# MPEGGroup/mpeg-pcc-tmc2

Measured on AMD Instinct MI355X. Metric: encoder patch+image-gen frames/sec, longdress_vox10 32-frame GOF, higher is better.
Workload: dtype int32/f64

## Files before the change

### mpeg-pcc-tmc2_amd/csrc/patches.hip

```cpp
#include <algorithm>
#include <cmath>

#include "internal.h"
#include "union_find.h"

namespace tmc2 {
namespace {

using Uf = UnionFind<false>;

constexpr uint32_t kNoLabel = 0xFFFFFFFFu;
constexpr uint32_t kFar     = 0xFFFFFFFFu;

struct PatchDev {
  int32_t u1, v1, d1;
  int32_t sizeU, sizeV, sizeU0, sizeV0;
  int32_t axN, axT, axB, mode;
  int32_t blockBase;
  int64_t depthOff;
  int64_t occOff;
};

__device__ __forceinline__ int coordOf( const Pt p, int axis ) { return axis == 0 ? p.x : ( axis == 1 ? p.y : p.z ); }

// ... 35 lines not shown
  for ( int j = 0; j < K; ++j ) {
    const uint32_t v = nb[j];
    if ( v == u ) continue;
    const uint4* rv  = reinterpret_cast<const uint4*>( knn + size_t( v ) * K );
    bool         hit = false;
#pragma unroll
    for ( int t = 0; t < K / 4; ++t ) {
      const uint4 r = rv[t];
      hit |= ( r.x == u ) | ( r.y == u ) | ( r.z == u ) | ( r.w == u );
    }
    m |= hit ? ( 1u << j ) : 0u;
  }
  mutual[u] = uint16_t( m );
}

template <int K>
__global__ __launch_bounds__( 256 ) void ccInitKernel( const uint32_t* __restrict__ knn, const uint16_t* __restrict__ mutual,
                                                        const uint8_t* __restrict__ partition, const uint8_t* __restrict__ raw,
                                                        const uint32_t* __restrict__ perm, bool chunked, uint32_t n,
                                                        uint32_t* __restrict__ parent, uint32_t* __restrict__ lab,
                                                        uint32_t* __restrict__ ccCount ) {
  const uint32_t i = pointOfLane( perm, chunked, n );
  if ( i >= n ) return;
  lab[i]        = kNoLabel;
  ccCount[i]    = 0;
  uint32_t best = i;
  if ( raw[i] ) {
    uint32_t      bestPrio = ufPriority( i ), m = mutual[i];
    const uint8_t pi       = partition[i];
    while ( m ) {
      const int j = __ffs( int( m ) ) - 1;
      m &= m - 1;
      const uint32_t v = knn[size_t( i ) * K + j];
      if ( ufPriority( v ) < bestPrio && raw[v] && partition[v] == pi ) {
        best     = v;
        bestPrio = ufPriority( v );
      }
    }
  }
  parent[i] = best;
}

template <int K>
__global__ __launch_bounds__( 256 ) void ccUnionKernel( const uint32_t* __restrict__ knn, const uint16_t* __restrict__ mutual,
                                                         const uint8_t* __restrict__ partition,
                                                         const uint8_t* __restrict__ raw, const uint32_t* __restrict__ perm,
                                                         bool chunked, uint32_t n, uint32_t* __restrict__ parent, int precheck,
                                                         bool agent ) {
  const uint32_t u = pointOfLane( perm, chunked, n );
  if ( u >= n || !raw[u] ) return;
  uint32_t m = mutual[u];
  if ( !m ) return;
  const uint8_t   pu  = partition[u];
  const uint32_t* row = knn + size_t( u ) * K;
  while ( m ) {
    const int j = __ffs( int( m ) ) - 1;
    m &= m - 1;
    const uint32_t v = row[j];
    if ( v > u || !raw[v] || partition[v] != pu ) continue;
    if ( precheck && Uf::sameSetStale( parent, u, v, agent ) ) continue;
    Uf::unite( parent, u, v, 0u, agent );
  }
}

template <int K>
__global__ __launch_bounds__( 256 ) void ccCheckKernel( const uint32_t* __restrict__ knn, const uint16_t* __restrict__ mutual,
                                                         const uint8_t* __restrict__ partition, const uint8_t* __restrict__ raw,
                                                         uint32_t n, uint32_t* parent, uint32_t* __restrict__ bad ) {
  const uint32_t u = blockIdx.x * blockDim.x + threadIdx.x;
  if ( u >= n || !raw[u] ) return;
  const uint32_t p = __hip_atomic_load( &parent[u], __ATOMIC_RELAXED, __HIP_MEMORY_SCOPE_AGENT );
  if ( p != u && ( p >= n || !raw[p] || partition[p] != partition[u] || ufPriority( p ) >= ufPriority( u ) ) ) atomicAdd( &bad[0], 1u );
  const uint32_t ru = Uf::rootCoherent( parent, u, n );
  if ( ru == kUfBroken ) {
    atomicAdd( &bad[0], 1u );
    return;
  }
  uint32_t m = mutual[u];
  while ( m ) {
    const int j = __ffs( int( m ) ) - 1;
    m &= m - 1;
    const uint32_t v = knn[size_t( u ) * K + j];
    if ( v > u || !raw[v] || partition[v] != partition[u] ) continue;
    if ( Uf::rootCoherent( parent, v, n ) != ru ) atomicAdd( &bad[1], 1u );
  }
}

__global__ __launch_bounds__( 256 ) void ccFlattenSeedKernel( const uint8_t* __restrict__ raw, const uint32_t* __restrict__ dist,
                                                               uint32_t thrDetection, uint32_t n,
                                                               uint32_t* __restrict__ parent, uint32_t* __restrict__ root,
                                                               uint32_t* __restrict__ lab, bool agent ) {
  const uint32_t u    = chunkedIndex();
  const int      lane = threadIdx.x & 63;
  uint32_t       r    = kNoLabel;
  bool           seed = false;
  if ( u < n && raw[u] ) {
    r       = Uf::find( parent, u, agent ).root;
    root[u] = r;
    seed    = dist[u] > thrDetection;
  }
  unsigned long long todo = __ballot( seed );
  while ( todo ) {
    const int                leader = __ffsll( (long long)todo ) - 1;
    const uint32_t           key    = __shfl( r, leader, 64 );
    const unsigned long long same   = __ballot( seed && r == key );
    if ( lane == leader && loadStaleOk( &lab[key], agent ) > u )
      atomicMin( &lab[key], u );
    todo &= ~same;
  }
}

template <int K>
__global__ __launch_bounds__( 256 ) void ccRelaxKernel( const uint32_t* __restrict__ knn, const uint16_t* __restrict__ mutual,
                                                         const uint8_t* __restrict__ partition,
                                                         const uint8_t* __restrict__ raw, const uint32_t* __restrict__ parent,
                                                         const uint32_t* __restrict__ perm, bool chunked, uint32_t n,
                                                         uint32_t* __restrict__ lab, uint32_t* __restrict__ changed, uint32_t token,
                                                         bool agent ) {
  const uint32_t u = pointOfLane( perm, chunked, n );
  if ( u >= n || !raw[u] ) return;
  uint32_t m = ~uint32_t( mutual[u] ) & ( ( 1u << K ) - 1u );
  if ( !m ) return;
  const uint32_t ru = parent[u];
  const uint32_t lu = loadStaleOk( &lab[ru], agent );
  if ( lu == kNoLabel ) return;
  const uint8_t   pu  = partition[u];
  const uint32_t* row = knn + size_t( u ) * K;
  bool            any = false;
  while ( m ) {
    const int j = __ffs( int( m ) ) - 1;
    m &= m - 1;
    const uint32_t v = row[j];
    if ( v == u || !raw[v] || partition[v] != pu ) continue;
    const uint32_t rv = parent[v];
    if ( rv != ru && loadStaleOk( &lab[rv], agent ) > lu &&
         atomicMin( &lab[rv], lu ) > lu )
      any = true;
  }
  if ( any ) *changed = token;
}

constexpr uint32_t kRawCounters = 16;
__global__ __launch_bounds__( 256 ) void patchBoundsInitKernel( uint32_t P, int32_t* __restrict__ bbox, int32_t* __restrict__ minUv,
                                                                 int32_t* __restrict__ patchStat, uint32_t* __restrict__ rawCount ) {
  const uint32_t p = blockIdx.x * blockDim.x + threadIdx.x;
  if ( p < kRawCounters ) rawCount[p * 32] = 0;
  if ( p >= P ) return;
#pragma unroll
  for ( int d = 0; d < 3; ++d ) {
    bbox[6 * p + d]     = 0x7FFFFFFF;
    bbox[6 * p + 3 + d] = 0;
  }
  minUv[2 * p] = minUv[2 * p + 1] = 0x7F7F7F7F;
  patchStat[2 * p] = patchStat[2 * p + 1] = 0;
}

__global__ __launch_bounds__( 256 ) void ccLabelCountKernel( const uint8_t* __restrict__ raw, const uint32_t* __restrict__ parent,
                                                              const uint32_t* __restrict__ lab, uint32_t n, uint32_t minCount,
                                                              uint32_t* __restrict__ label, uint32_t* __restrict__ ccCount ) {
  const uint32_t i    = chunkedIndex();
  const int      lane = threadIdx.x & 63;
  const uint32_t l    = ( i < n && raw[i] ) ? lab[parent[i]] : kNoLabel;
  if ( i < n ) label[i] = l;
  unsigned long long todo = __ballot( l != kNoLabel );
  while ( todo ) {
    const int                leader = __ffsll( (long long)todo ) - 1;
    const uint32_t           key    = __shfl( l, leader, 64 );
    const unsigned long long same   = __ballot( l == key );
    if ( lane == leader && loadStaleOk( &ccCount[key] ) < minCount ) atomicAdd( &ccCount[key], uint32_t( __popcll( same ) ) );
    todo &= ~same;
  }
}

__global__ __launch_bounds__( 256 ) void ccSeedFlagKernel( const uint32_t* __restrict__ label,
                                                            const uint32_t* __restrict__ ccCount, uint32_t minCount,
                                                            uint32_t n, uint32_t* __restrict__ flag ) {
  const uint32_t i = chunkedIndex();
  if ( i < n ) flag[i] = ( label[i] == i && ccCount[i] >= minCount ) ? 1u : 0u;
}

__global__ __launch_bounds__( 256 ) void ccAssignKernel( const uint32_t* __restrict__ label,
                                                          const uint32_t* __restrict__ ccCount,
                                                          const uint32_t* __restrict__ rank,
                                                          const uint8_t* __restrict__ partition, uint32_t minCount,
                                                          uint32_t n, int32_t* __restrict__ pointPatch,
                                                          int32_t* __restrict__ patchView ) {
  const uint32_t i = chunkedIndex();
  if ( i >= n ) return;
  const uint32_t l = label[i];
  int32_t        p = -1;
  if ( l != kNoLabel && ccCount[l] >= minCount ) {
    p = int32_t( rank[l] );
    if ( l == i ) patchView[p] = partition[i];
  }
  pointPatch[i] = p;
}

constexpr int kAggSlots = 128;
template <int FIELDS>
struct PatchAgg {
  int32_t key[kAggSlots];
  int32_t val[kAggSlots][FIELDS];
};
template <int FIELDS, int MINS>
__device__ __forceinline__ void aggInit( PatchAgg<FIELDS>& t ) {
  for ( int i = threadIdx.x; i < kAggSlots; i += blockDim.x ) {
    t.key[i] = -1;
// ... 28 lines not shown
}
template <int FIELDS, int MINS>
__device__ __forceinline__ void aggFlush( PatchAgg<FIELDS>& t, int32_t* __restrict__ out ) {
  __syncthreads();
  for ( int i = threadIdx.x; i < kAggSlots * FIELDS; i += blockDim.x ) {
    const int     slot = i / FIELDS, f = i % FIELDS;
    const int32_t k    = t.key[slot];
    if ( k < 0 ) continue;
    if ( f < MINS )
      lazyAtomicMin( &out[FIELDS * k + f], t.val[slot][f] );
    else
      lazyAtomicMax( &out[FIELDS * k + f], t.val[slot][f] );
  }
}

__global__ __launch_bounds__( 256 ) void patchMinUvKernel( const Pt* __restrict__ pts, const int32_t* __restrict__ pointPatch,
                                                            const int32_t* __restrict__ patchView, uint32_t n,
                                                            int32_t* __restrict__ minUv ) {
  __shared__ PatchAgg<2> agg;
  aggInit<2, 2>( agg );
  const uint32_t i = chunkedIndex();
  const int32_t  p = i < n ? pointPatch[i] : -1;
  if ( p >= 0 ) {
    const int view = patchView[p] % 3;
    const int axT = view == 0 ? 2 : ( view == 1 ? 2 : 0 ), axB = view == 0 ? 1 : ( view == 1 ? 0 : 1 );
    const Pt  q    = pts[i];
    const int uv[2] = {coordOf( q, axT ), coordOf( q, axB )};
    aggAdd<2, 2>( agg, p, uv, minUv );
  }
  aggFlush<2, 2>( agg, minUv );
}

__global__ __launch_bounds__( 256 ) void patchTrimBboxKernel( const Pt* __restrict__ pts, const int32_t* __restrict__ patchView,
                                                               const int32_t* __restrict__ minUv, int splitting,
                                                               int maxPatchSize, uint32_t n,
                                                               int32_t* __restrict__ pointPatch, int32_t* __restrict__ bbox ) {
  __shared__ PatchAgg<6> agg;
  aggInit<6, 3>( agg );
  const uint32_t i = chunkedIndex();
  int32_t        p = i < n ? pointPatch[i] : -1;
  if ( p >= 0 ) {
    const Pt q = pts[i];
    if ( splitting ) {
      const int view = patchView[p] % 3;
      const int axT = view == 0 ? 2 : ( view == 1 ? 2 : 0 ), axB = view == 0 ? 1 : ( view == 1 ? 0 : 1 );
      if ( !( coordOf( q, axT ) - minUv[2 * p] < maxPatchSize && coordOf( q, axB ) - minUv[2 * p + 1] < maxPatchSize ) ) {
        pointPatch[i] = -1;
        p             = -1;
      }
    }
    if ( p >= 0 ) {
      const int box[6] = {q.x, q.y, q.z, q.x, q.y, q.z};
      aggAdd<6, 3>( agg, p, box, bbox );
    }
  }
  aggFlush<6, 3>( agg, bbox );
}

__global__ __launch_bounds__( 256 ) void patchDepth0Kernel( const Pt* __restrict__ pts, const int32_t* __restrict__ pointPatch,
                                                             const PatchDev* __restrict__ patches, uint32_t n,
                                                             int64_t roundDepthBase,
                                                             unsigned long long* __restrict__ map64 ) {
  const uint32_t i = chunkedIndex();
  if ( i >= n ) return;
  const int32_t p = pointPatch[i];
  if ( p < 0 ) return;
  const PatchDev pd = patches[p];
  const Pt       q  = pts[i];
  const int      d = coordOf( q, pd.axN ), u = coordOf( q, pd.axT ) - pd.u1, v = coordOf( q, pd.axB ) - pd.v1;
  const size_t   px  = size_t( pd.depthOff - roundDepthBase ) + size_t( v ) * pd.sizeU + u;
  const unsigned long long val = ( (unsigned long long)uint32_t( d + 1 ) << 32 ) | i;
  if ( pd.mode == 0 )
    atomicMin( &map64[px], val );
  else
    atomicMax( &map64[px], val );
}

__global__ __launch_bounds__( 256 ) void patchInitTileKernel( const PatchDev* __restrict__ patches,
// ... 50 lines not shown
  if ( depth != INF ) {
    const int     dir = 1 - 2 * pd.mode;
    const int16_t a   = int16_t( abs( depth - pk ) );
    const int16_t b   = int16_t( int16_t( surfaceThickness ) + dir * depth );
    const int16_t c   = int16_t( dir * pd.d1 + int16_t( maxAllowedDepth ) );
    if ( a > 32 || b > c ) {
      depth = INF;
      src   = 0xFFFFFFFFu;
    }
  }
  d0tmp[px] = depth;
  d1tmp[px] = depth;
  d0src[px] = src;
}

__global__ __launch_bounds__( 256 ) void patchDepth1Kernel( const Pt* __restrict__ pts, const uint8_t* __restrict__ rgb4,
                                                             const int32_t* __restrict__ pointPatch,
                                                             const PatchDev* __restrict__ patches, uint32_t n,
                                                             int64_t roundDepthBase, int surfaceThickness,
                                                             const int32_t* __restrict__ d0tmp,
                                                             const uint32_t* __restrict__ d0src, int32_t* __restrict__ d1tmp ) {
  const uint32_t i = chunkedIndex();
  if ( i >= n ) return;
  const int32_t p = pointPatch[i];
  if ( p < 0 ) return;
  const PatchDev pd = patches[p];
  const Pt       q  = pts[i];
  const int      d = coordOf( q, pd.axN ), u = coordOf( q, pd.axT ) - pd.u1, v = coordOf( q, pd.axB ) - pd.v1;
  const size_t   px = size_t( pd.depthOff - roundDepthBase ) + size_t( v ) * pd.sizeU + u;
  const int      z0 = d0tmp[px];
  if ( !( z0 < 32767 ) ) return;
  const int     dir   = 1 - 2 * pd.mode;
  const int16_t delta = int16_t( dir * ( d - z0 ) );
  if ( !( delta <= int16_t( surfaceThickness ) && delta >= 0 ) ) return;
  const uchar4 ci = reinterpret_cast<const uchar4*>( rgb4 )[i];
  const uchar4 c0 = reinterpret_cast<const uchar4*>( rgb4 )[d0src[px]];
  if ( !( abs( int( c0.x ) - int( ci.x ) ) < 128 && abs( int( c0.y ) - int( ci.y ) ) < 128 &&
// ... 58 lines not shown
    anyValid[threadIdx.x >> 6] = __popcll( m );
    tileMax[threadIdx.x >> 6]  = mx;
  }
  __syncthreads();
  if ( threadIdx.x == 0 ) {
    const int count = anyValid[0] + anyValid[1] + anyValid[2] + anyValid[3];
    occupancy[size_t( pd.occOff ) + size_t( bv ) * pd.sizeU0 + bu] = count ? 1 : 0;
    if ( count ) {
      const int tmx = max( max( tileMax[0], tileMax[1] ), max( tileMax[2], tileMax[3] ) );
      if ( tmx > loadStaleOk( &patchStat[2 * p] ) ) atomicMax( &patchStat[2 * p], tmx );
      atomicAdd( &patchStat[2 * p + 1], count );
    }
  }
}

__global__ __launch_bounds__( 256 ) void rawDistanceKernel( const Pt* __restrict__ pts, uint32_t n,
                                                             const uint32_t* __restrict__ bitmap, int bitmapBits,
                                                             const int* __restrict__ offsets, int nOffsets,
                                                             uint32_t thrSelection, uint32_t* __restrict__ dist,
                                                             uint8_t* __restrict__ raw, uint32_t* __restrict__ rawCount ) {
  const uint32_t i = chunkedIndex();
  bool           isRaw = false;
  if ( i < n ) {
    const Pt  q    = pts[i];
    const int size = 1 << bitmapBits;
    uint32_t  best = kFar;
    for ( int o = 0; o < nOffsets; ++o ) {
      const int packed = offsets[o];
      const int dx = ( packed & 0xFF ) - 128, dy = ( ( packed >> 8 ) & 0xFF ) - 128, dz = ( ( packed >> 16 ) & 0xFF ) - 128;
      const int x = q.x + dx, y = q.y + dy, z = q.z + dz;
      if ( x < 0 || y < 0 || z < 0 || x >= size || y >= size || z >= size ) continue;
      const size_t bit = size_t( x ) + ( size_t( y ) << bitmapBits ) + ( size_t( z ) << ( 2 * bitmapBits ) );
      if ( bitmap[bit >> 5] & ( 1u << ( bit & 31 ) ) ) {
        best = uint32_t( packed >> 24 );
        break;
      }
    }
    dist[i] = best;
    isRaw   = best > thrSelection;
    raw[i]  = isRaw ? 1 : 0;
  }
  __shared__ uint32_t wgRaw;
  if ( threadIdx.x == 0 ) wgRaw = 0;
  __syncthreads();
  const unsigned long long m = __ballot( isRaw );
  if ( ( threadIdx.x & 63 ) == 0 && m ) atomicAdd( &wgRaw, uint32_t( __popcll( m ) ) );
  __syncthreads();
  if ( threadIdx.x == 0 && wgRaw ) atomicAdd( &rawCount[( blockIdx.x % kRawCounters ) * 32], wgRaw );
}

}

int ensureMutualMask( tmc2_frame* f ) {
  if ( f->haveMutual ) return TMC2_OK;
  const uint32_t n = uint32_t( f->n );
  TMC2_TRY( f->d_mutual.alloc( n ) );
  StageScope stage( f->ctx, "k:ccMutualMask" );
  const PassOrder order  = passOrder( f, "MUTUAL_ORDER" );
  const uint32_t  blocks = ( n + 255 ) / 256;
  hipLaunchKernelGGL( ccMutualMaskKernel<16>, dim3( order.chunked ? chunkedGrid( blocks ) : blocks ), dim3( 256 ), 0, f->ctx->stream, f->d_knn.p,
                      order.perm, order.chunked, n, f->d_mutual.p );
  TMC2_HIP( hipGetLastError() );
  f->haveMutual = true;
// ... 36 lines not shown
    std::vector<std::pair<int, int>> tmp;
    for ( int dz = -R; dz <= R; ++dz )
      for ( int dy = -R; dy <= R; ++dy )
        for ( int dx = -R; dx <= R; ++dx ) {
          const int d2 = dx * dx + dy * dy + dz * dz;
          if ( d2 <= probeR2 ) tmp.emplace_back( d2, ( dx + 128 ) | ( ( dy + 128 ) << 8 ) | ( ( dz + 128 ) << 16 ) );
        }
    std::sort( tmp.begin(), tmp.end() );
    for ( auto& t : tmp ) offsets.push_back( t.second | ( t.first << 24 ) );
  }
  int bitmapBits = 1;
  while ( ( 1 << bitmapBits ) <= int( f->geoMax ) ) ++bitmapBits;
  const size_t bitmapWords = ( size_t( 1 ) << ( 3 * bitmapBits ) ) >> 5;
  TMC2_TRY( ctx->voxelBitmap.alloc( bitmapWords ) );

  DevBuf<uint32_t> d_label, d_ccCount, d_flag, d_rank, d_dist, d_small, d_tilePatch, d_d0src, d_parent, d_root, d_lab;
  DevBuf<uint8_t>  d_raw;
  DevBuf<int32_t>  d_pointPatch, d_minUv, d_bbox, d_patchStat, d_d0tmp, d_d1tmp;
  DevBuf<PatchDev> d_patches;
  DevBuf<unsigned long long> d_map64;
  TMC2_TRY( d_label.alloc( n ) );
  TMC2_TRY( d_parent.alloc( n ) );
  TMC2_TRY( d_root.alloc( n ) );
  TMC2_TRY( d_lab.alloc( n ) );
  TMC2_TRY( d_ccCount.alloc( n ) );
  TMC2_TRY( d_flag.alloc( n ) );
  TMC2_TRY( d_rank.alloc( n ) );
  TMC2_TRY( d_dist.alloc( n ) );
  TMC2_TRY( d_raw.alloc( n ) );
  TMC2_TRY( d_pointPatch.alloc( n ) );
  TMC2_TRY( d_small.alloc( 16 ) );
  const int* d_offsets = ctx->constTable( ( uint64_t( 0x5339 ) << 32 ) | uint64_t( probeR2 ), offsets );
  if ( !d_offsets ) return TMC2_E_HIP;
  TMC2_TRY( fillRegions( ctx, {{ctx->voxelBitmap.p, bitmapWords * 4, 0},
                               {d_raw.p, n, 1},
                               {d_dist.p, size_t( n ) * 4, 0xFF},
                               {d_small.p, 64, 0}} ) );

  f->patches.clear();
  f->patchesChanged();
  f->depthCount = 0;
  f->occCount   = 0;
  const dim3  blk( 256 ), grdN( chunkedGrid( ( n + 255 ) / 256 ) );
  uint32_t    rawCount = n, relaxToken = 0;
  int        rounds   = 0;
  TMC2_TRY( ensureMutualMask( f ) );
  DevBuf<uint16_t>& d_mutual   = f->d_mutual;
  const bool        agentScope = unionAgentScope( f->ctx );
  const PassOrder order   = passOrder( f, "MUTUAL_ORDER" );
  const bool      chunked = order.chunked;
  const uint32_t* perm    = order.perm;
  while ( rawCount > 0 ) {
    StageScope cc( ctx, "patches_cc" );
    hipLaunchKernelGGL( ccInitKernel<16>, grdN, blk, 0, s, f->d_knn.p, d_mutual.p, f->d_partition.p, d_raw.p, perm, chunked, n, d_parent.p,
                        d_lab.p, d_ccCount.p );
    {
      StageScope kt( ctx, "k:ccUnion" );
      hipLaunchKernelGGL( ccUnionKernel<16>, grdN, blk, 0, s, f->d_knn.p, d_mutual.p, f->d_partition.p, d_raw.p, perm, chunked, n,
                          d_parent.p, unionPrecheck( f->ctx ), agentScope );
      kt.end();
      if ( unionCheck( f->ctx ) ) {
        TMC2_HIP( hipMemsetAsync( d_small.p + 8, 0, 8, s ) );
        hipLaunchKernelGGL( ccCheckKernel<16>, grdN, blk, 0, s, f->d_knn.p, d_mutual.p, f->d_partition.p, d_raw.p, n,
                            d_parent.p, d_small.p + 8 );
        TMC2_TRY( unionCheckResult( s, d_small.p + 8, "segmentPatches: union-find invariant broken in round " + std::to_string( rounds ) ) );
      }
      hipLaunchKernelGGL( ccFlattenSeedKernel, grdN, blk, 0, s, d_raw.p, d_dist.p, thrDet, n, d_parent.p, d_root.p, d_lab.p,
                          agentScope );
    }
    uint32_t P = 0;
    for ( int guard = 0; guard < 1 << 20; ++guard ) {
      StageScope kt( ctx, "k:ccRelax" );
      for ( int b = 0; b < 3; ++b )
        hipLaunchKernelGGL( ccRelaxKernel<16>, grdN, blk, 0, s, f->d_knn.p, d_mutual.p, f->d_partition.p, d_raw.p,
                            d_root.p, perm, chunked, n, d_lab.p, d_small.p, ++relaxToken, agentScope );
      kt.end();
      hipLaunchKernelGGL( ccLabelCountKernel, grdN, blk, 0, s, d_raw.p, d_root.p, d_lab.p, n,
                          uint32_t( sp->minPointCountPerCCPatchSegmentation ), d_label.p, d_ccCount.p );
      hipLaunchKernelGGL( ccSeedFlagKernel, grdN, blk, 0, s, d_label.p, d_ccCount.p,
                          uint32_t( sp->minPointCountPerCCPatchSegmentation ), n, d_flag.p );
      volatile uint32_t* answer = ctx->answerLine( tmc2_ctx::kAnswerPatchRound );
      TMC2_TRY( exclusiveScanU32( ctx, d_flag.p, d_rank.p, n, d_small.p + 1, ScanAnswer{answer, d_small.p, 1} ) );
      TMC2_HIP( hipStreamSynchronize( s ) );
      P = answer[0];
      if ( answer[1] != relaxToken ) break;
      TMC2_HIP( hipMemsetAsync( d_ccCount.p, 0, size_t( n ) * 4, s ) );
    }
    cc.end();
    if ( P == 0 ) break;
    StageScope build( ctx, "patches_build" );
    TMC2_TRY( d_minUv.alloc( 2 * size_t( P ) ) );
    TMC2_TRY( d_bbox.alloc( 7 * size_t( P ) ) );
    const size_t statWords = 2 * size_t( P ) + size_t( kRawCounters ) * 32;
    TMC2_TRY( d_patchStat.alloc( statWords ) );
    int32_t*  d_view     = d_bbox.p + 6 * size_t( P );
    uint32_t* d_rawCount = reinterpret_cast<uint32_t*>( d_patchStat.p + 2 * size_t( P ) );
    TMC2_TRY( d_patches.alloc( P ) );
    hipLaunchKernelGGL( ccAssignKernel, grdN, blk, 0, s, d_label.p, d_ccCount.p, d_rank.p, f->d_partition.p,
                        uint32_t( sp->minPointCountPerCCPatchSegmentation ), n, d_pointPatch.p, d_view );
    hipLaunchKernelGGL( patchBoundsInitKernel, dim3( ( P + 255 ) / 256 ), blk, 0, s, P, d_bbox.p, d_minUv.p, d_patchStat.p,
                        d_rawCount );
    if ( sp->enablePatchSplitting )
      hipLaunchKernelGGL( patchMinUvKernel, grdN, blk, 0, s, f->d_pts.p, d_pointPatch.p, d_view, n, d_minUv.p );
    hipLaunchKernelGGL( patchTrimBboxKernel, grdN, blk, 0, s, f->d_pts.p, d_view, d_minUv.p,
                        sp->enablePatchSplitting, sp->maxPatchSize, n, d_pointPatch.p, d_bbox.p );
    int32_t* h_records = ctx->hostRecords.get<int32_t>( std::max<size_t>( 7 * size_t( P ) + statWords, size_t( 1 ) << 16 ) );
    if ( !h_records ) {
      setError( "segmentPatches: hipHostMalloc failed" );
      return TMC2_E_HIP;
    }
    const int32_t* h_bbox = h_records;
    TMC2_HIP( hipMemcpyAsync( h_records, d_bbox.p, 7 * size_t( P ) * 4, hipMemcpyDeviceToHost, s ) );
    const int32_t* h_view = h_bbox + 6 * size_t( P );
    TMC2_HIP( hipStreamSynchronize( s ) );
    for ( uint32_t p = 0; p < P; ++p )
      if ( h_bbox[6 * p] > h_bbox[6 * p + 3] ) {
        f->patches.clear();
        f->depthCount = f->occCount = 0;
        f->havePatches              = false;
        setError( "segmentPatches: patch splitting with maxPatchSize=%d keeps no point of a connected component (round %d); "
// ... 51 lines not shown
    const size_t pdBytes = ( size_t( P ) * sizeof( PatchDev ) + 15 ) & ~size_t( 15 );
    uint8_t*     h_tables = ctx->hostTables.get<uint8_t>( std::max<size_t>( pdBytes + size_t( tiles ) * 4, size_t( 1 ) << 20 ) );
    if ( !h_tables ) {
      setError( "segmentPatches: hipHostMalloc failed" );
      return TMC2_E_HIP;
    }
    memcpy( h_tables, h_pd, size_t( P ) * sizeof( PatchDev ) );
    uint32_t* h_tilePatch = reinterpret_cast<uint32_t*>( h_tables + pdBytes );
    for ( uint32_t p = 0, at = 0; p < P; ++p )
      for ( uint32_t b = uint32_t( h_pd[p].sizeU0 ) * uint32_t( h_pd[p].sizeV0 ); b > 0; --b ) h_tilePatch[at++] = p;
    TMC2_TRY( f->growPools() );
    TMC2_TRY( d_map64.alloc( roundArea ) );
    TMC2_TRY( d_d0tmp.alloc( roundArea ) );
    TMC2_TRY( d_d1tmp.alloc( roundArea ) );
    TMC2_TRY( d_d0src.alloc( roundArea ) );
    TMC2_TRY( d_tilePatch.alloc( tiles ) );
    TMC2_HIP( hipMemcpyAsync( d_patches.p, h_tables, size_t( P ) * sizeof( PatchDev ), hipMemcpyHostToDevice, s ) );
    TMC2_HIP( hipMemcpyAsync( d_tilePatch.p, h_tilePatch, size_t( tiles ) * 4, hipMemcpyHostToDevice, s ) );
    hipLaunchKernelGGL( patchInitTileKernel, dim3( tiles ), blk, 0, s, d_patches.p, d_tilePatch.p, roundDepthBase, occRes,
                        d_map64.p );
    hipLaunchKernelGGL( patchDepth0Kernel, grdN, blk, 0, s, f->d_pts.p, d_pointPatch.p, d_patches.p, n, roundDepthBase,
                        d_map64.p );
    hipLaunchKernelGGL( patchFilterTileKernel, dim3( tiles ), blk, 0, s, d_patches.p, d_tilePatch.p, d_map64.p,
                        roundDepthBase, occRes, sp->surfaceThickness, sp->maxAllowedDepth, d_d0tmp.p, d_d1tmp.p,
                        d_d0src.p );
    if ( sp->surfaceThickness > 0 )
      hipLaunchKernelGGL( patchDepth1Kernel, grdN, blk, 0, s, f->d_pts.p, f->d_rgb.p, d_pointPatch.p, d_patches.p, n,
                          roundDepthBase, sp->surfaceThickness, d_d0tmp.p, d_d0src.p, d_d1tmp.p );
    hipLaunchKernelGGL( patchResampleTileKernel, dim3( tiles ), blk, 0, s, d_patches.p, d_tilePatch.p, roundDepthBase,
                        occRes, d_d0tmp.p, d_d1tmp.p, bitmapBits, ctx->voxelBitmap.p, f->d_depth0.p, f->d_depth1.p,
                        f->d_occupancy.p, d_patchStat.p );
    int32_t* h_stat = h_records + 7 * size_t( P );
    hipLaunchKernelGGL( rawDistanceKernel, grdN, blk, 0, s, f->d_pts.p, n, ctx->voxelBitmap.p, bitmapBits, d_offsets,
                        int( offsets.size() ), thrSel, d_dist.p, d_raw.p, d_rawCount );
    TMC2_HIP( hipMemcpyAsync( h_stat, d_patchStat.p, statWords * 4, hipMemcpyDeviceToHost, s ) );
    TMC2_HIP( hipStreamSynchronize( s ) );
    const uint32_t rawBefore = rawCount;
    rawCount = 0;
    for ( uint32_t c = 0; c < kRawCounters; ++c ) rawCount += uint32_t( h_stat[2 * size_t( P ) + size_t( c ) * 32] );
    build.end();
    if ( rawCount >= rawBefore ) {
      f->patches.clear();
      f->depthCount = f->occCount = 0;
      f->havePatches              = false;
      setError( "segmentPatches: round %d took no point off the raw list (%u left); the reference does not terminate on this input",
                rounds, rawCount );
      return TMC2_E_UNSUPPORTED;
    }
    for ( uint32_t p = 0; p < P; ++p ) {
      tmc2_patch& T = f->patches[patchBase + p];
      const int   sizeD = h_stat[2 * p];
      T.sizeDPixel      = sizeD;
      const int bits    = std::min( sp->geometryBitDepth3D, sp->geometryBitDepth2D );
      const int L       = sp->minLevel;
      const int sd      = std::min( ( 1 << bits ) - 1, sizeD );
      const int bitsD   = bits - int( std::log2( L ) );
      int       q       = sd == 0 ? 0 : ( ( sd - 1 ) / L + 1 );
      q                 = std::min( q, ( 1 << bitsD ) - 1 );
      T.sizeD           = q == 0 ? 0 : ( q * L - 1 );
      T.d0Count         = h_stat[2 * p + 1];
      T.eomAndD1Count   = 0;
    }
    ++rounds;
  }
  TMC2_HIP( hipGetLastError() );
  f->rounds      = rounds;
  f->havePatches = true;
  f->geometryBitDepth3D = sp->geometryBitDepth3D;
  return TMC2_OK;
}

}

extern "C" int tmc2_selftest_components( tmc2_ctx* ctx, const uint32_t* d_knn, const uint8_t* d_partition, const uint8_t* d_raw,
                                         const uint32_t* d_perm, uint64_t n64, uint32_t* d_root, uint32_t* d_bad ) {
  using namespace tmc2;
  if ( !ctx || !d_knn || !d_partition || !d_raw || !d_root || !d_bad || n64 == 0 || n64 > 0x0FFFFFFFull ) {
    setError( "selftest_components: invalid argument (null pointer, no point, or more than 2^28 - 1 points)" );
    return TMC2_E_INVALID;
// ... 6 lines not shown
  TMC2_TRY( d_mutual.alloc( n ) );
  TMC2_TRY( d_parent.alloc( n ) );
  TMC2_TRY( d_lab.alloc( n ) );
  TMC2_TRY( d_ccCount.alloc( n ) );
  TMC2_TRY( d_dist.alloc( n ) );
  TMC2_TRY( fillRegions( ctx, {{d_parent.p, size_t( n ) * 4, 0}, {d_mutual.p, size_t( n ) * 2, 0}, {d_dist.p, size_t( n ) * 4, 0}} ) );
  const auto      option  = ctxOption( ctx, "MUTUAL_ORDER" );
  const char      o       = option ? ( *option )[0] : 'c';
  const bool      chunked = o != 'i';
  const uint32_t* perm    = o == 't' ? d_perm : nullptr;
  const uint32_t  blocks  = ( n + 255 ) / 256;
  const dim3      blk( 256 ), grdN( chunkedGrid( blocks ) );
  const bool      agentScope = unionAgentScope( ctx );
  hipLaunchKernelGGL( ccMutualMaskKernel<16>, dim3( chunked ? chunkedGrid( blocks ) : blocks ), dim3( 256 ), 0, s, d_knn, perm, chunked, n,
                      d_mutual.p );
  hipLaunchKernelGGL( ccInitKernel<16>, grdN, blk, 0, s, d_knn, d_mutual.p, d_partition, d_raw, perm, chunked, n, d_parent.p, d_lab.p,
                      d_ccCount.p );
  hipLaunchKernelGGL( ccUnionKernel<16>, grdN, blk, 0, s, d_knn, d_mutual.p, d_partition, d_raw, perm, chunked, n, d_parent.p,
                      unionPrecheck( ctx ), agentScope );
  if ( unionCheck( ctx ) )
    hipLaunchKernelGGL( ccCheckKernel<16>, grdN, blk, 0, s, d_knn, d_mutual.p, d_partition, d_raw, n, d_parent.p, d_bad );
  hipLaunchKernelGGL( ccFlattenSeedKernel, grdN, blk, 0, s, d_raw, d_dist.p, 0xFFFFFFFFu, n, d_parent.p, d_root, d_lab.p, agentScope );
  TMC2_HIP( hipGetLastError() );
  return TMC2_OK;
}
```

Before: 194.8.

## Compact raw points into a list so later segmentation rounds process only them

After each patch round, raw points are compacted through a flag scan and scatter into a ping-pong list with a position map. Later rounds launch the CC, assignment, bbox, depth and raw-distance kernels over that list only, not all n points. The per-block raw counters are replaced by a scan total read from a host-visible answer line, and the patch and tile tables are merged into one upload. This cuts work in rounds after the first, at the cost of an extra scan and scatter per round, indirect indexing, and added bookkeeping complexity.

```diff
diff --git a/mpeg-pcc-tmc2_amd/csrc/patches.hip b/mpeg-pcc-tmc2_amd/csrc/patches.hip
--- a/mpeg-pcc-tmc2_amd/csrc/patches.hip
+++ b/mpeg-pcc-tmc2_amd/csrc/patches.hip
@@ -73,13 +73,26 @@
   mutual[u] = uint16_t( m );
 }
 
-template <int K>
+template <bool LIST>
+__device__ __forceinline__ uint32_t roundPoint( const uint32_t* __restrict__ list, uint32_t count, uint32_t n ) {
+  const uint32_t j = chunkedIndex();
+  if ( LIST ) return j < count ? list[j] : n;
+  return j < n ? j : n;
+}
+template <bool LIST>
+__device__ __forceinline__ uint32_t roundPoint( const uint32_t* __restrict__ list, uint32_t count, const uint32_t* __restrict__ perm,
+                                                bool chunked, uint32_t n ) {
+  return LIST ? roundPoint<true>( list, count, n ) : pointOfLane( perm, chunked, n );
+}
+
+template <bool LIST, int K>
 __global__ __launch_bounds__( 256 ) void ccInitKernel( const uint32_t* __restrict__ knn, const uint16_t* __restrict__ mutual,
                                                         const uint8_t* __restrict__ partition, const uint8_t* __restrict__ raw,
-                                                        const uint32_t* __restrict__ perm, bool chunked, uint32_t n,
+                                                        const uint32_t* __restrict__ perm, bool chunked,
+                                                        const uint32_t* __restrict__ list, uint32_t count, uint32_t n,
                                                         uint32_t* __restrict__ parent, uint32_t* __restrict__ lab,
                                                         uint32_t* __restrict__ ccCount ) {
-  const uint32_t i = pointOfLane( perm, chunked, n );
+  const uint32_t i = roundPoint<LIST>( list, count, perm, chunked, n );
   if ( i >= n ) return;
   lab[i]        = kNoLabel;
   ccCount[i]    = 0;
@@ -100,13 +113,13 @@
   parent[i] = best;
 }
 
-template <int K>
+template <bool LIST, int K>
 __global__ __launch_bounds__( 256 ) void ccUnionKernel( const uint32_t* __restrict__ knn, const uint16_t* __restrict__ mutual,
                                                          const uint8_t* __restrict__ partition,
                                                          const uint8_t* __restrict__ raw, const uint32_t* __restrict__ perm,
-                                                         bool chunked, uint32_t n, uint32_t* __restrict__ parent, int precheck,
-                                                         bool agent ) {
-  const uint32_t u = pointOfLane( perm, chunked, n );
+                                                         bool chunked, const uint32_t* __restrict__ list, uint32_t count, uint32_t n,
+                                                         uint32_t* __restrict__ parent, int precheck, bool agent ) {
+  const uint32_t u = roundPoint<LIST>( list, count, perm, chunked, n );
   if ( u >= n || !raw[u] ) return;
   uint32_t m = mutual[u];
   if ( !m ) return;
@@ -122,11 +135,14 @@
   }
 }
 
-template <int K>
+template <bool LIST, int K>
 __global__ __launch_bounds__( 256 ) void ccCheckKernel( const uint32_t* __restrict__ knn, const uint16_t* __restrict__ mutual,
                                                          const uint8_t* __restrict__ partition, const uint8_t* __restrict__ raw,
-                                                         uint32_t n, uint32_t* parent, uint32_t* __restrict__ bad ) {
-  const uint32_t u = blockIdx.x * blockDim.x + threadIdx.x;
+                                                         const uint32_t* __restrict__ list, uint32_t count, uint32_t n, uint32_t* parent,
+                                                         uint32_t* __restrict__ bad ) {
+  const uint32_t at = blockIdx.x * blockDim.x + threadIdx.x;
+  if ( at >= count ) return;
+  const uint32_t u = LIST ? list[at] : at;
   if ( u >= n || !raw[u] ) return;
   const uint32_t p = __hip_atomic_load( &parent[u], __ATOMIC_RELAXED, __HIP_MEMORY_SCOPE_AGENT );
   if ( p != u && ( p >= n || !raw[p] || partition[p] != partition[u] || ufPriority( p ) >= ufPriority( u ) ) ) atomicAdd( &bad[0], 1u );
@@ -145,11 +161,12 @@
   }
 }
 
+template <bool LIST>
 __global__ __launch_bounds__( 256 ) void ccFlattenSeedKernel( const uint8_t* __restrict__ raw, const uint32_t* __restrict__ dist,
-                                                               uint32_t thrDetection, uint32_t n,
-                                                               uint32_t* __restrict__ parent, uint32_t* __restrict__ root,
-                                                               uint32_t* __restrict__ lab, bool agent ) {
-  const uint32_t u    = chunkedIndex();
+                                                               uint32_t thrDetection, const uint32_t* __restrict__ list,
+                                                               uint32_t count, uint32_t n, uint32_t* __restrict__ parent,
+                                                               uint32_t* __restrict__ root, uint32_t* __restrict__ lab, bool agent ) {
+  const uint32_t u    = roundPoint<LIST>( list, count, n );
   const int      lane = threadIdx.x & 63;
   uint32_t       r    = kNoLabel;
   bool           seed = false;
@@ -169,14 +186,15 @@
   }
 }
 
-template <int K>
+template <bool LIST, int K>
 __global__ __launch_bounds__( 256 ) void ccRelaxKernel( const uint32_t* __restrict__ knn, const uint16_t* __restrict__ mutual,
                                                          const uint8_t* __restrict__ partition,
                                                          const uint8_t* __restrict__ raw, const uint32_t* __restrict__ parent,
-                                                         const uint32_t* __restrict__ perm, bool chunked, uint32_t n,
+                                                         const uint32_t* __restrict__ perm, bool chunked,
+                                                         const uint32_t* __restrict__ list, uint32_t count, uint32_t n,
                                                          uint32_t* __restrict__ lab, uint32_t* __restrict__ changed, uint32_t token,
                                                          bool agent ) {
-  const uint32_t u = pointOfLane( perm, chunked, n );
+  const uint32_t u = roundPoint<LIST>( list, count, perm, chunked, n );
   if ( u >= n || !raw[u] ) return;
   uint32_t m = ~uint32_t( mutual[u] ) & ( ( 1u << K ) - 1u );
   if ( !m ) return;
@@ -199,11 +217,9 @@
   if ( any ) *changed = token;
 }
 
-constexpr uint32_t kRawCounters = 16;
 __global__ __launch_bounds__( 256 ) void patchBoundsInitKernel( uint32_t P, int32_t* __restrict__ bbox, int32_t* __restrict__ minUv,
-                                                                 int32_t* __restrict__ patchStat, uint32_t* __restrict__ rawCount ) {
+                                                                 int32_t* __restrict__ patchStat ) {
   const uint32_t p = blockIdx.x * blockDim.x + threadIdx.x;
-  if ( p < kRawCounters ) rawCount[p * 32] = 0;
   if ( p >= P ) return;
 #pragma unroll
   for ( int d = 0; d < 3; ++d ) {
@@ -214,10 +230,12 @@
   patchStat[2 * p] = patchStat[2 * p + 1] = 0;
 }
 
+template <bool LIST>
 __global__ __launch_bounds__( 256 ) void ccLabelCountKernel( const uint8_t* __restrict__ raw, const uint32_t* __restrict__ parent,
-                                                              const uint32_t* __restrict__ lab, uint32_t n, uint32_t minCount,
+                                                              const uint32_t* __restrict__ lab, const uint32_t* __restrict__ list,
+                                                              uint32_t count, uint32_t n, uint32_t minCount,
                                                               uint32_t* __restrict__ label, uint32_t* __restrict__ ccCount ) {
-  const uint32_t i    = chunkedIndex();
+  const uint32_t i    = roundPoint<LIST>( list, count, n );
   const int      lane = threadIdx.x & 63;
   const uint32_t l    = ( i < n && raw[i] ) ? lab[parent[i]] : kNoLabel;
   if ( i < n ) label[i] = l;
@@ -231,25 +249,36 @@
   }
 }
 
+__global__ __launch_bounds__( 256 ) void ccClearCountKernel( const uint32_t* __restrict__ list, uint32_t count,
+                                                              uint32_t* __restrict__ ccCount ) {
+  const uint32_t j = chunkedIndex();
+  if ( j < count ) ccCount[list[j]] = 0;
+}
+
+template <bool LIST>
 __global__ __launch_bounds__( 256 ) void ccSeedFlagKernel( const uint32_t* __restrict__ label,
                                                             const uint32_t* __restrict__ ccCount, uint32_t minCount,
-                                                            uint32_t n, uint32_t* __restrict__ flag ) {
-  const uint32_t i = chunkedIndex();
-  if ( i < n ) flag[i] = ( label[i] == i && ccCount[i] >= minCount ) ? 1u : 0u;
-}
-
+                                                            const uint32_t* __restrict__ list, uint32_t count,
+                                                            uint32_t* __restrict__ flag ) {
+  const uint32_t j = chunkedIndex();
+  if ( j >= count ) return;
+  const uint32_t i = LIST ? list[j] : j;
+  flag[j]          = ( label[i] == i && ccCount[i] >= minCount ) ? 1u : 0u;
+}
+
+template <bool LIST>
 __global__ __launch_bounds__( 256 ) void ccAssignKernel( const uint32_t* __restrict__ label,
                                                           const uint32_t* __restrict__ ccCount,
-                                                          const uint32_t* __restrict__ rank,
+                                                          const uint32_t* __restrict__ rank, const uint32_t* __restrict__ posOf,
                                                           const uint8_t* __restrict__ partition, uint32_t minCount,
-                                                          uint32_t n, int32_t* __restrict__ pointPatch,
-                                                          int32_t* __restrict__ patchView ) {
-  const uint32_t i = chunkedIndex();
+                                                          const uint32_t* __restrict__ list, uint32_t count, uint32_t n,
+                                                          int32_t* __restrict__ pointPatch, int32_t* __restrict__ patchView ) {
+  const uint32_t i = roundPoint<LIST>( list, count, n );
   if ( i >= n ) return;
   const uint32_t l = label[i];
   int32_t        p = -1;
   if ( l != kNoLabel && ccCount[l] >= minCount ) {
-    p = int32_t( rank[l] );
+    p = int32_t( rank[LIST ? posOf[l] : l] );
     if ( l == i ) patchView[p] = partition[i];
   }
   pointPatch[i] = p;
@@ -308,12 +337,13 @@
   }
 }
 
+template <bool LIST>
 __global__ __launch_bounds__( 256 ) void patchMinUvKernel( const Pt* __restrict__ pts, const int32_t* __restrict__ pointPatch,
-                                                            const int32_t* __restrict__ patchView, uint32_t n,
-                                                            int32_t* __restrict__ minUv ) {
+                                                            const int32_t* __restrict__ patchView, const uint32_t* __restrict__ list,
+                                                            uint32_t count, uint32_t n, int32_t* __restrict__ minUv ) {
   __shared__ PatchAgg<2> agg;
   aggInit<2, 2>( agg );
-  const uint32_t i = chunkedIndex();
+  const uint32_t i = roundPoint<LIST>( list, count, n );
   const int32_t  p = i < n ? pointPatch[i] : -1;
   if ( p >= 0 ) {
     const int view = patchView[p] % 3;
@@ -325,13 +355,15 @@
   aggFlush<2, 2>( agg, minUv );
 }
 
+template <bool LIST>
 __global__ __launch_bounds__( 256 ) void patchTrimBboxKernel( const Pt* __restrict__ pts, const int32_t* __restrict__ patchView,
                                                                const int32_t* __restrict__ minUv, int splitting,
-                                                               int maxPatchSize, uint32_t n,
-                                                               int32_t* __restrict__ pointPatch, int32_t* __restrict__ bbox ) {
+                                                               int maxPatchSize, const uint32_t* __restrict__ list, uint32_t count,
+                                                               uint32_t n, int32_t* __restrict__ pointPatch,
+                                                               int32_t* __restrict__ bbox ) {
   __shared__ PatchAgg<6> agg;
   aggInit<6, 3>( agg );
-  const uint32_t i = chunkedIndex();
+  const uint32_t i = roundPoint<LIST>( list, count, n );
   int32_t        p = i < n ? pointPatch[i] : -1;
   if ( p >= 0 ) {
     const Pt q = pts[i];
@@ -351,11 +383,12 @@
   aggFlush<6, 3>( agg, bbox );
 }
 
+template <bool LIST>
 __global__ __launch_bounds__( 256 ) void patchDepth0Kernel( const Pt* __restrict__ pts, const int32_t* __restrict__ pointPatch,
-                                                             const PatchDev* __restrict__ patches, uint32_t n,
-                                                             int64_t roundDepthBase,
+                                                             const PatchDev* __restrict__ patches, const uint32_t* __restrict__ list,
+                                                             uint32_t count, uint32_t n, int64_t roundDepthBase,
                                                              unsigned long long* __restrict__ map64 ) {
-  const uint32_t i = chunkedIndex();
+  const uint32_t i = roundPoint<LIST>( list, count, n );
   if ( i >= n ) return;
   const int32_t p = pointPatch[i];
   if ( p < 0 ) return;
@@ -436,13 +469,14 @@
   d0src[px] = src;
 }
 
+template <bool LIST>
 __global__ __launch_bounds__( 256 ) void patchDepth1Kernel( const Pt* __restrict__ pts, const uint8_t* __restrict__ rgb4,
                                                              const int32_t* __restrict__ pointPatch,
-                                                             const PatchDev* __restrict__ patches, uint32_t n,
-                                                             int64_t roundDepthBase, int surfaceThickness,
+                                                             const PatchDev* __restrict__ patches, const uint32_t* __restrict__ list,
+                                                             uint32_t count, uint32_t n, int64_t roundDepthBase, int surfaceThickness,
                                                              const int32_t* __restrict__ d0tmp,
                                                              const uint32_t* __restrict__ d0src, int32_t* __restrict__ d1tmp ) {
-  const uint32_t i = chunkedIndex();
+  const uint32_t i = roundPoint<LIST>( list, count, n );
   if ( i >= n ) return;
   const int32_t p = pointPatch[i];
   if ( p < 0 ) return;
@@ -531,39 +565,44 @@
   }
 }
 
-__global__ __launch_bounds__( 256 ) void rawDistanceKernel( const Pt* __restrict__ pts, uint32_t n,
+template <bool LIST>
+__global__ __launch_bounds__( 256 ) void rawDistanceKernel( const Pt* __restrict__ pts, const uint32_t* __restrict__ list, uint32_t count,
                                                              const uint32_t* __restrict__ bitmap, int bitmapBits,
                                                              const int* __restrict__ offsets, int nOffsets,
                                                              uint32_t thrSelection, uint32_t* __restrict__ dist,
-                                                             uint8_t* __restrict__ raw, uint32_t* __restrict__ rawCount ) {
-  const uint32_t i = chunkedIndex();
-  bool           isRaw = false;
-  if ( i < n ) {
-    const Pt  q    = pts[i];
-    const int size = 1 << bitmapBits;
-    uint32_t  best = kFar;
-    for ( int o = 0; o < nOffsets; ++o ) {
-      const int packed = offsets[o];
-      const int dx = ( packed & 0xFF ) - 128, dy = ( ( packed >> 8 ) & 0xFF ) - 128, dz = ( ( packed >> 16 ) & 0xFF ) - 128;
-      const int x = q.x + dx, y = q.y + dy, z = q.z + dz;
-      if ( x < 0 || y < 0 || z < 0 || x >= size || y >= size || z >= size ) continue;
-      const size_t bit = size_t( x ) + ( size_t( y ) << bitmapBits ) + ( size_t( z ) << ( 2 * bitmapBits ) );
-      if ( bitmap[bit >> 5] & ( 1u << ( bit & 31 ) ) ) {
-        best = uint32_t( packed >> 24 );
-        break;
-      }
-    }
-    dist[i] = best;
-    isRaw   = best > thrSelection;
-    raw[i]  = isRaw ? 1 : 0;
-  }
-  __shared__ uint32_t wgRaw;
-  if ( threadIdx.x == 0 ) wgRaw = 0;
-  __syncthreads();
-  const unsigned long long m = __ballot( isRaw );
-  if ( ( threadIdx.x & 63 ) == 0 && m ) atomicAdd( &wgRaw, uint32_t( __popcll( m ) ) );
-  __syncthreads();
-  if ( threadIdx.x == 0 && wgRaw ) atomicAdd( &rawCount[( blockIdx.x % kRawCounters ) * 32], wgRaw );
+                                                             uint8_t* __restrict__ raw, uint32_t* __restrict__ keep ) {
+  const uint32_t j = chunkedIndex();
+  if ( j >= count ) return;
+  const uint32_t i    = LIST ? list[j] : j;
+  const Pt       q    = pts[i];
+  const int      size = 1 << bitmapBits;
+  uint32_t       best = kFar;
+  for ( int o = 0; o < nOffsets; ++o ) {
+    const int packed = offsets[o];
+    const int dx = ( packed & 0xFF ) - 128, dy = ( ( packed >> 8 ) & 0xFF ) - 128, dz = ( ( packed >> 16 ) & 0xFF ) - 128;
+    const int x = q.x + dx, y = q.y + dy, z = q.z + dz;
+    if ( x < 0 || y < 0 || z < 0 || x >= size || y >= size || z >= size ) continue;
+    const size_t bit = size_t( x ) + ( size_t( y ) << bitmapBits ) + ( size_t( z ) << ( 2 * bitmapBits ) );
+    if ( bitmap[bit >> 5] & ( 1u << ( bit & 31 ) ) ) {
+      best = uint32_t( packed >> 24 );
+      break;
+    }
+  }
+  const bool isRaw = best > thrSelection;
+  dist[i]          = best;
+  raw[i]           = isRaw ? 1 : 0;
+  keep[j]          = isRaw ? 1u : 0u;
+}
+
+template <bool LIST>
+__global__ __launch_bounds__( 256 ) void rawListScatterKernel( const uint32_t* __restrict__ list, uint32_t count,
+                                                                const uint32_t* __restrict__ keep, const uint32_t* __restrict__ pos,
+                                                                uint32_t* __restrict__ next, uint32_t* __restrict__ posOf ) {
+  const uint32_t j = chunkedIndex();
+  if ( j >= count || !keep[j] ) return;
+  const uint32_t i = LIST ? list[j] : j;
+  next[pos[j]]     = i;
+  posOf[i]         = pos[j];
 }
 
 }
@@ -630,10 +669,9 @@
   const size_t bitmapWords = ( size_t( 1 ) << ( 3 * bitmapBits ) ) >> 5;
   TMC2_TRY( ctx->voxelBitmap.alloc( bitmapWords ) );
 
-  DevBuf<uint32_t> d_label, d_ccCount, d_flag, d_rank, d_dist, d_small, d_tilePatch, d_d0src, d_parent, d_root, d_lab;
-  DevBuf<uint8_t>  d_raw;
+  DevBuf<uint32_t> d_label, d_ccCount, d_flag, d_rank, d_dist, d_small, d_d0src, d_parent, d_root, d_lab, d_rawList[2], d_posOf;
+  DevBuf<uint8_t>  d_raw, d_tables;
   DevBuf<int32_t>  d_pointPatch, d_minUv, d_bbox, d_patchStat, d_d0tmp, d_d1tmp;
-  DevBuf<PatchDev> d_patches;
   DevBuf<unsigned long long> d_map64;
   TMC2_TRY( d_label.alloc( n ) );
   TMC2_TRY( d_parent.alloc( n ) );
@@ -645,6 +683,9 @@
   TMC2_TRY( d_dist.alloc( n ) );
   TMC2_TRY( d_raw.alloc( n ) );
   TMC2_TRY( d_pointPatch.alloc( n ) );
+  TMC2_TRY( d_rawList[0].alloc( n ) );
+  TMC2_TRY( d_rawList[1].alloc( n ) );
+  TMC2_TRY( d_posOf.alloc( n ) );
   TMC2_TRY( d_small.alloc( 16 ) );
   const int* d_offsets = ctx->constTable( ( uint64_t( 0x5339 ) << 32 ) | uint64_t( probeR2 ), offsets );
   if ( !d_offsets ) return TMC2_E_HIP;
@@ -666,60 +707,67 @@
   const PassOrder order   = passOrder( f, "MUTUAL_ORDER" );
   const bool      chunked = order.chunked;
   const uint32_t* perm    = order.perm;
-  while ( rawCount > 0 ) {
+  const uint32_t  minCount = uint32_t( sp->minPointCountPerCCPatchSegmentation );
+#define ROUND_KERNEL( name, ... ) ( listed ? name<true, ##__VA_ARGS__> : name<false, ##__VA_ARGS__> )
+  bool listed = false;
+  int  cur    = 0;
+  while ( rawCount > 0 && rawCount >= minCount ) {
+    const uint32_t* list  = listed ? d_rawList[cur].p : nullptr;
+    const uint32_t  count = rawCount;
+    const dim3      grd   = listed ? dim3( chunkedGrid( ( count + 255 ) / 256 ) ) : grdN;
     StageScope cc( ctx, "patches_cc" );
-    hipLaunchKernelGGL( ccInitKernel<16>, grdN, blk, 0, s, f->d_knn.p, d_mutual.p, f->d_partition.p, d_raw.p, perm, chunked, n, d_parent.p,
-                        d_lab.p, d_ccCount.p );
+    hipLaunchKernelGGL( ROUND_KERNEL( ccInitKernel, 16 ), grd, blk, 0, s, f->d_knn.p, d_mutual.p, f->d_partition.p, d_raw.p, perm, chunked,
+                        list, count, n, d_parent.p, d_lab.p, d_ccCount.p );
     {
       StageScope kt( ctx, "k:ccUnion" );
-      hipLaunchKernelGGL( ccUnionKernel<16>, grdN, blk, 0, s, f->d_knn.p, d_mutual.p, f->d_partition.p, d_raw.p, perm, chunked, n,
-                          d_parent.p, unionPrecheck( f->ctx ), agentScope );
+      hipLaunchKernelGGL( ROUND_KERNEL( ccUnionKernel, 16 ), grd, blk, 0, s, f->d_knn.p, d_mutual.p, f->d_partition.p, d_raw.p, perm,
+                          chunked, list, count, n, d_parent.p, unionPrecheck( f->ctx ), agentScope );
       kt.end();
       if ( unionCheck( f->ctx ) ) {
         TMC2_HIP( hipMemsetAsync( d_small.p + 8, 0, 8, s ) );
-        hipLaunchKernelGGL( ccCheckKernel<16>, grdN, blk, 0, s, f->d_knn.p, d_mutual.p, f->d_partition.p, d_raw.p, n,
-                            d_parent.p, d_small.p + 8 );
+        hipLaunchKernelGGL( ROUND_KERNEL( ccCheckKernel, 16 ), grd, blk, 0, s, f->d_knn.p, d_mutual.p, f->d_partition.p, d_raw.p, list,
+                            count, n, d_parent.p, d_small.p + 8 );
         TMC2_TRY( unionCheckResult( s, d_small.p + 8, "segmentPatches: union-find invariant broken in round " + std::to_string( rounds ) ) );
       }
-      hipLaunchKernelGGL( ccFlattenSeedKernel, grdN, blk, 0, s, d_raw.p, d_dist.p, thrDet, n, d_parent.p, d_root.p, d_lab.p,
-                          agentScope );
+      hipLaunchKernelGGL( ROUND_KERNEL( ccFlattenSeedKernel ), grd, blk, 0, s, d_raw.p, d_dist.p, thrDet, list, count, n, d_parent.p,
+                          d_root.p, d_lab.p, agentScope );
     }
     uint32_t P = 0;
     for ( int guard = 0; guard < 1 << 20; ++guard ) {
       StageScope kt( ctx, "k:ccRelax" );
       for ( int b = 0; b < 3; ++b )
-        hipLaunchKernelGGL( ccRelaxKernel<16>, grdN, blk, 0, s, f->d_knn.p, d_mutual.p, f->d_partition.p, d_raw.p,
-                            d_root.p, perm, chunked, n, d_lab.p, d_small.p, ++relaxToken, agentScope );
+        hipLaunchKernelGGL( ROUND_KERNEL( ccRelaxKernel, 16 ), grd, blk, 0, s, f->d_knn.p, d_mutual.p, f->d_partition.p, d_raw.p,
+                            d_root.p, perm, chunked, list, count, n, d_lab.p, d_small.p, ++relaxToken, agentScope );
       kt.end();
-      hipLaunchKernelGGL( ccLabelCountKernel, grdN, blk, 0, s, d_raw.p, d_root.p, d_lab.p, n,
-                          uint32_t( sp->minPointCountPerCCPatchSegmentation ), d_label.p, d_ccCount.p );
-      hipLaunchKernelGGL( ccSeedFlagKernel, grdN, blk, 0, s, d_label.p, d_ccCount.p,
-                          uint32_t( sp->minPointCountPerCCPatchSegmentation ), n, d_flag.p );
+      hipLaunchKernelGGL( ROUND_KERNEL( ccLabelCountKernel ), grd, blk, 0, s, d_raw.p, d_root.p, d_lab.p, list, count, n, minCount,
+                          d_label.p, d_ccCount.p );
+      hipLaunchKernelGGL( ROUND_KERNEL( ccSeedFlagKernel ), grd, blk, 0, s, d_label.p, d_ccCount.p, minCount, list, count, d_flag.p );
       volatile uint32_t* answer = ctx->answerLine( tmc2_ctx::kAnswerPatchRound );
-      TMC2_TRY( exclusiveScanU32( ctx, d_flag.p, d_rank.p, n, d_small.p + 1, ScanAnswer{answer, d_small.p, 1} ) );
+      TMC2_TRY( exclusiveScanU32( ctx, d_flag.p, d_rank.p, count, d_small.p + 1, ScanAnswer{answer, d_small.p, 1} ) );
       TMC2_HIP( hipStreamSynchronize( s ) );
       P = answer[0];
       if ( answer[1] != relaxToken ) break;
-      TMC2_HIP( hipMemsetAsync( d_ccCount.p, 0, size_t( n ) * 4, s ) );
+      if ( listed )
+        hipLaunchKernelGGL( ccClearCountKernel, grd, blk, 0, s, list, count, d_ccCount.p );
+      else
+        TMC2_HIP( hipMemsetAsync( d_ccCount.p, 0, size_t( n ) * 4, s ) );
     }
     cc.end();
     if ( P == 0 ) break;
     StageScope build( ctx, "patches_build" );
     TMC2_TRY( d_minUv.alloc( 2 * size_t( P ) ) );
     TMC2_TRY( d_bbox.alloc( 7 * size_t( P ) ) );
-    const size_t statWords = 2 * size_t( P ) + size_t( kRawCounters ) * 32;
+    const size_t statWords = 2 * size_t( P );
     TMC2_TRY( d_patchStat.alloc( statWords ) );
-    int32_t*  d_view     = d_bbox.p + 6 * size_t( P );
-    uint32_t* d_rawCount = reinterpret_cast<uint32_t*>( d_patchStat.p + 2 * size_t( P ) );
-    TMC2_TRY( d_patches.alloc( P ) );
-    hipLaunchKernelGGL( ccAssignKernel, grdN, blk, 0, s, d_label.p, d_ccCount.p, d_rank.p, f->d_partition.p,
-                        uint32_t( sp->minPointCountPerCCPatchSegmentation ), n, d_pointPatch.p, d_view );
-    hipLaunchKernelGGL( patchBoundsInitKernel, dim3( ( P + 255 ) / 256 ), blk, 0, s, P, d_bbox.p, d_minUv.p, d_patchStat.p,
-                        d_rawCount );
+    int32_t* d_view = d_bbox.p + 6 * size_t( P );
+    hipLaunchKernelGGL( ROUND_KERNEL( ccAssignKernel ), grd, blk, 0, s, d_label.p, d_ccCount.p, d_rank.p, d_posOf.p, f->d_partition.p,
+                        minCount, list, count, n, d_pointPatch.p, d_view );
+    hipLaunchKernelGGL( patchBoundsInitKernel, dim3( ( P + 255 ) / 256 ), blk, 0, s, P, d_bbox.p, d_minUv.p, d_patchStat.p );
     if ( sp->enablePatchSplitting )
-      hipLaunchKernelGGL( patchMinUvKernel, grdN, blk, 0, s, f->d_pts.p, d_pointPatch.p, d_view, n, d_minUv.p );
-    hipLaunchKernelGGL( patchTrimBboxKernel, grdN, blk, 0, s, f->d_pts.p, d_view, d_minUv.p,
-                        sp->enablePatchSplitting, sp->maxPatchSize, n, d_pointPatch.p, d_bbox.p );
+      hipLaunchKernelGGL( ROUND_KERNEL( patchMinUvKernel ), grd, blk, 0, s, f->d_pts.p, d_pointPatch.p, d_view, list, count, n,
+                          d_minUv.p );
+    hipLaunchKernelGGL( ROUND_KERNEL( patchTrimBboxKernel ), grd, blk, 0, s, f->d_pts.p, d_view, d_minUv.p, sp->enablePatchSplitting,
+                        sp->maxPatchSize, list, count, n, d_pointPatch.p, d_bbox.p );
     int32_t* h_records = ctx->hostRecords.get<int32_t>( std::max<size_t>( 7 * size_t( P ) + statWords, size_t( 1 ) << 16 ) );
     if ( !h_records ) {
       setError( "segmentPatches: hipHostMalloc failed" );
@@ -801,30 +849,37 @@
     TMC2_TRY( d_d0tmp.alloc( roundArea ) );
     TMC2_TRY( d_d1tmp.alloc( roundArea ) );
     TMC2_TRY( d_d0src.alloc( roundArea ) );
-    TMC2_TRY( d_tilePatch.alloc( tiles ) );
-    TMC2_HIP( hipMemcpyAsync( d_patches.p, h_tables, size_t( P ) * sizeof( PatchDev ), hipMemcpyHostToDevice, s ) );
-    TMC2_HIP( hipMemcpyAsync( d_tilePatch.p, h_tilePatch, size_t( tiles ) * 4, hipMemcpyHostToDevice, s ) );
-    hipLaunchKernelGGL( patchInitTileKernel, dim3( tiles ), blk, 0, s, d_patches.p, d_tilePatch.p, roundDepthBase, occRes,
-                        d_map64.p );
-    hipLaunchKernelGGL( patchDepth0Kernel, grdN, blk, 0, s, f->d_pts.p, d_pointPatch.p, d_patches.p, n, roundDepthBase,
-                        d_map64.p );
-    hipLaunchKernelGGL( patchFilterTileKernel, dim3( tiles ), blk, 0, s, d_patches.p, d_tilePatch.p, d_map64.p,
-                        roundDepthBase, occRes, sp->surfaceThickness, sp->maxAllowedDepth, d_d0tmp.p, d_d1tmp.p,
-                        d_d0src.p );
+    TMC2_TRY( d_tables.alloc( pdBytes + size_t( tiles ) * 4 ) );
+    const PatchDev* d_patches   = reinterpret_cast<const PatchDev*>( d_tables.p );
+    const uint32_t* d_tilePatch = reinterpret_cast<const uint32_t*>( d_tables.p + pdBytes );
+    TMC2_HIP( hipMemcpyAsync( d_tables.p, h_tables, pdBytes + size_t( tiles ) * 4, hipMemcpyHostToDevice, s ) );
+    hipLaunchKernelGGL( patchInitTileKernel, dim3( tiles ), blk, 0, s, d_patches, d_tilePatch, roundDepthBase, occRes, d_map64.p );
+    hipLaunchKernelGGL( ROUND_KERNEL( patchDepth0Kernel ), grd, blk, 0, s, f->d_pts.p, d_pointPatch.p, d_patches, list, count, n,
+                        roundDepthBase, d_map64.p );
+    hipLaunchKernelGGL( patchFilterTileKernel, dim3( tiles ), blk, 0, s, d_patches, d_tilePatch, d_map64.p, roundDepthBase, occRes,
+                        sp->surfaceThickness, sp->maxAllowedDepth, d_d0tmp.p, d_d1tmp.p, d_d0src.p );
     if ( sp->surfaceThickness > 0 )
-      hipLaunchKernelGGL( patchDepth1Kernel, grdN, blk, 0, s, f->d_pts.p, f->d_rgb.p, d_pointPatch.p, d_patches.p, n,
-                          roundDepthBase, sp->surfaceThickness, d_d0tmp.p, d_d0src.p, d_d1tmp.p );
-    hipLaunchKernelGGL( patchResampleTileKernel, dim3( tiles ), blk, 0, s, d_patches.p, d_tilePatch.p, roundDepthBase,
-                        occRes, d_d0tmp.p, d_d1tmp.p, bitmapBits, ctx->voxelBitmap.p, f->d_depth0.p, f->d_depth1.p,
-                        f->d_occupancy.p, d_patchStat.p );
+      hipLaunchKernelGGL( ROUND_KERNEL( patchDepth1Kernel ), grd, blk, 0, s, f->d_pts.p, f->d_rgb.p, d_pointPatch.p, d_patches, list,
+                          count, n, roundDepthBase, sp->surfaceThickness, d_d0tmp.p, d_d0src.p, d_d1tmp.p );
+    hipLaunchKernelGGL( patchResampleTileKernel, dim3( tiles ), blk, 0, s, d_patches, d_tilePatch, roundDepthBase, occRes, d_d0tmp.p,
+                        d_d1tmp.p, bitmapBits, ctx->voxelBitmap.p, f->d_depth0.p, f->d_depth1.p, f->d_occupancy.p, d_patchStat.p );
     int32_t* h_stat = h_records + 7 * size_t( P );
-    hipLaunchKernelGGL( rawDistanceKernel, grdN, blk, 0, s, f->d_pts.p, n, ctx->voxelBitmap.p, bitmapBits, d_offsets,
-                        int( offsets.size() ), thrSel, d_dist.p, d_raw.p, d_rawCount );
+    volatile uint32_t* answer = ctx->answerLine( tmc2_ctx::kAnswerPatchRound );
+    hipLaunchKernelGGL( ROUND_KERNEL( rawDistanceKernel ), grd, blk, 0, s, f->d_pts.p, list, count, ctx->voxelBitmap.p, bitmapBits,
+                        d_offsets, int( offsets.size() ), thrSel, d_dist.p, d_raw.p, d_flag.p );
+    const int scanned = exclusiveScanU32( ctx, d_flag.p, d_rank.p, count, nullptr, ScanAnswer{answer, nullptr, 0} );
+    if ( scanned != TMC2_OK ) {
+      (void)hipStreamSynchronize( s );
+      return scanned;
+    }
+    hipLaunchKernelGGL( ROUND_KERNEL( rawListScatterKernel ), grd, blk, 0, s, list, count, d_flag.p, d_rank.p, d_rawList[cur ^ 1].p,
+                        d_posOf.p );
     TMC2_HIP( hipMemcpyAsync( h_stat, d_patchStat.p, statWords * 4, hipMemcpyDeviceToHost, s ) );
     TMC2_HIP( hipStreamSynchronize( s ) );
     const uint32_t rawBefore = rawCount;
-    rawCount = 0;
-    for ( uint32_t c = 0; c < kRawCounters; ++c ) rawCount += uint32_t( h_stat[2 * size_t( P ) + size_t( c ) * 32] );
+    rawCount                 = answer[0];
+    cur ^= 1;
+    listed = true;
     build.end();
     if ( rawCount >= rawBefore ) {
       f->patches.clear();
@@ -850,6 +905,7 @@
     }
     ++rounds;
   }
+#undef ROUND_KERNEL
   TMC2_HIP( hipGetLastError() );
   f->rounds      = rounds;
   f->havePatches = true;
@@ -886,13 +942,16 @@
   const bool      agentScope = unionAgentScope( ctx );
   hipLaunchKernelGGL( ccMutualMaskKernel<16>, dim3( chunked ? chunkedGrid( blocks ) : blocks ), dim3( 256 ), 0, s, d_knn, perm, chunked, n,
                       d_mutual.p );
-  hipLaunchKernelGGL( ccInitKernel<16>, grdN, blk, 0, s, d_knn, d_mutual.p, d_partition, d_raw, perm, chunked, n, d_parent.p, d_lab.p,
-                      d_ccCount.p );
-  hipLaunchKernelGGL( ccUnionKernel<16>, grdN, blk, 0, s, d_knn, d_mutual.p, d_partition, d_raw, perm, chunked, n, d_parent.p,
-                      unionPrecheck( ctx ), agentScope );
+  const uint32_t* noList = nullptr;
+  hipLaunchKernelGGL( ( ccInitKernel<false, 16> ), grdN, blk, 0, s, d_knn, d_mutual.p, d_partition, d_raw, perm, chunked, noList, n, n,
+                      d_parent.p, d_lab.p, d_ccCount.p );
+  hipLaunchKernelGGL( ( ccUnionKernel<false, 16> ), grdN, blk, 0, s, d_knn, d_mutual.p, d_partition, d_raw, perm, chunked, noList, n, n,
+                      d_parent.p, unionPrecheck( ctx ), agentScope );
   if ( unionCheck( ctx ) )
-    hipLaunchKernelGGL( ccCheckKernel<16>, grdN, blk, 0, s, d_knn, d_mutual.p, d_partition, d_raw, n, d_parent.p, d_bad );
-  hipLaunchKernelGGL( ccFlattenSeedKernel, grdN, blk, 0, s, d_raw, d_dist.p, 0xFFFFFFFFu, n, d_parent.p, d_root, d_lab.p, agentScope );
+    hipLaunchKernelGGL( ( ccCheckKernel<false, 16> ), grdN, blk, 0, s, d_knn, d_mutual.p, d_partition, d_raw, noList, n, n, d_parent.p,
+                        d_bad );
+  hipLaunchKernelGGL( ccFlattenSeedKernel<false>, grdN, blk, 0, s, d_raw, d_dist.p, 0xFFFFFFFFu, noList, n, n, d_parent.p, d_root,
+                      d_lab.p, agentScope );
   TMC2_HIP( hipGetLastError() );
   return TMC2_OK;
 }
```

Measured after the change: 197.5, median of 6. 1.01x the previous value.
